# Fireflies-17/Speech-Inpainting

Measured on AMD Instinct MI355X. Metric: real-time factor (audio-sec/wall-sec) per GPU, 4 s clips @16 kHz, 200 ms mask, higher is better.
Workload: dtype encoder GEMMs and attention products: bf16 MFMA, fp32 accumulate (softmax, LayerNorm, head, arg-max in fp32); vocoder: fp16 MFMA (operands rounded to fp16, saturating), fp32 accumulate, activations stored as fp16; 1 GPU; BASELINE configs[1]: batch=32 x 4 s clips per GPU, 200 ms mask, HuBERT-base + HiFi-GAN V1; step = masked log-mel front-end -> encoder -> arg-max/splice -> vocoder on resident raw clips; global_batch=32, clip_samples=64000, mask_frames=10, parallelism=utterance-sharded x1

## Files before the change

speech_inpainting_amd/csrc/api.hip:

```cpp
#include <cmath>
#include <cstdarg>
#include <cstdio>
#include <cstdlib>
#include <cstring>
#include <map>
#include <sstream>
#include <string>
#include <vector>

#include "common.h"

namespace {

struct HostTensor {
    const float* data = nullptr;
    std::vector<long> shape;
    long numel() const { long n = 1; for (long d : shape) n *= d; return n; }
};

struct GemmW {
    size_t w = 0, w_lo = 0, bias = 0;
    int Cin = 0, N = 0, Npad = 0, ntaps = 0, groups = 1, math = 0;
    bool has_bias = false;
};

struct LayerW { GemmW qkv, out, ffn1, ffn2; size_t ln1_g, ln1_b, ln2_g, ln2_b; };
struct ConvW { GemmW g; size_t ln_g = 0, ln_b = 0; };
struct ResW { GemmW c1[SI_MAX_DIL], c2[SI_MAX_DIL]; };

struct Layout {
    size_t total = 0;
    size_t conv0_w, conv0_bias, conv0_g, conv0_b;
    std::vector<ConvW> convs;
    size_t fp_ln_g, fp_ln_b; GemmW proj;
    GemmW pos; size_t enc_ln_g, enc_ln_b;
    std::vector<LayerW> layers;
    size_t head_ln_g, head_ln_b; GemmW head;
    size_t cb_centered, cb_raw, cb_rnorm;
    GemmW pre; std::vector<GemmW> ups; std::vector<ResW> rbs;
    size_t post_w, post_b; int post_C = 0;
    int mel_ld = 0;
};

}

struct si_ctx {
    int device = 0;
    si_model_desc d{};
    char err[512] = {0};
    Layout lay;
    char* wdev = nullptr;
    bool weights_ready = false;
    bool weights_verified = false;
    std::map<std::string, long> dbg_size;
    std::map<std::string, std::pair<float*, long>> dbg_capture;
    struct ProfRec { int name; hipEvent_t a, b; double flops, bytes; };
    bool prof_on = false;
    std::string prof_filter;
    std::vector<std::string> prof_names;
    std::vector<ProfRec> prof_recs;
    std::vector<hipEvent_t> prof_pool;
    size_t prof_used = 0;
    int prof_open = -1;
    int num_cus = 0;
    std::map<const void*, size_t> dyn_lds;
    bool opt_voc_opready = true, opt_voc_res16 = true, opt_enc_opready = true, opt_att_bf16 = true, opt_enc_lingemm = true;
    bool opt_enc_posconv = true;
    int opt_ln_fuse = 1;
    int opt_voc_upsgemm = 1;
    int opt_ffn_pad = 64;
    int opt_gemmcu = 1;
    int opt_voc_chain = 1;
    int opt_voc_fuse = 1;
    char* fe_dev = nullptr;
    size_t fe_dft = 0, fe_hann = 0, fe_basis = 0, fe_lo = 0, fe_hi = 0;
    std::vector<int32_t> vl_host;
    static constexpr int VL_SLOTS = 4;
    int32_t* vl_pin[VL_SLOTS] = {nullptr, nullptr, nullptr, nullptr};
    size_t vl_pin_ints[VL_SLOTS] = {0, 0, 0, 0};
    hipEvent_t vl_ev[VL_SLOTS] = {nullptr, nullptr, nullptr, nullptr};
    int vl_next = 0;
    float* km_cnorm = nullptr;
    int km_cnorm_cap = 0;
};

static char g_create_err[512] = "";

int si_fail(si_ctx* ctx, int code, const char* fmt, ...) {
    char* dst = ctx ? ctx->err : g_create_err;
    va_list ap;
    va_start(ap, fmt);
    vsnprintf(dst, 512, fmt, ap);
    va_end(ap);
    return code;
}
int si_fail_hip(si_ctx* ctx, hipError_t e, const char* what, const char* file, int line) {
    return si_fail(ctx, SI_EHIP, "HIP error %d (%s) at %s:%d: %s", (int)e, hipGetErrorString(e), file, line, what);
}

struct TapSrc { const void* p; long n; int esize = 4; long cols = 0, ld = 0; };
static int si_tap(si_ctx* ctx, hipStream_t st, TapSrc s, const char* fmt, int a = 0, int b = 0, int c = 0) {
    if (ctx->dbg_capture.empty() && strchr(fmt, '%')) return SI_OK;
    char name[48];
    snprintf(name, sizeof(name), fmt, a, b, c);
    ctx->dbg_size[name] = s.n;
    auto it = ctx->dbg_capture.find(name);
    if (it == ctx->dbg_capture.end()) return SI_OK;
    const long m = s.n < it->second.second ? s.n : it->second.second;
    if (m <= 0) return SI_OK;
    if (s.ld > s.cols && s.cols > 0) {
        if (m / s.cols > 0)
            SI_HIP_CHECK(hipMemcpy2DAsync(it->second.first, (size_t)s.cols * s.esize, s.p, (size_t)s.ld * s.esize, (size_t)s.cols * s.esize,
                                          (size_t)(m / s.cols), hipMemcpyDeviceToDevice, st));
    } else {
        SI_HIP_CHECK(hipMemcpyAsync(it->second.first, s.p, (size_t)m * s.esize, hipMemcpyDeviceToDevice, st));
    }
    return SI_OK;
}

void si_prof_begin(si_ctx* ctx, const char* name, double flops, double bytes, hipStream_t st) {
    if (!ctx->prof_on || ctx->prof_used + 2 > ctx->prof_pool.size()) { ctx->prof_open = -1; return; }
    if (!ctx->prof_filter.empty() && ctx->prof_filter != name) { ctx->prof_open = -1; return; }
    int id = -1;
    for (size_t i = 0; i < ctx->prof_names.size(); ++i) if (ctx->prof_names[i] == name) { id = (int)i; break; }
    if (id < 0) { id = (int)ctx->prof_names.size(); ctx->prof_names.push_back(name); }
    si_ctx::ProfRec r{id, ctx->prof_pool[ctx->prof_used], ctx->prof_pool[ctx->prof_used + 1], flops, bytes};
    ctx->prof_used += 2;
    (void)hipEventRecord(r.a, st);
    ctx->prof_open = (int)ctx->prof_recs.size();
    ctx->prof_recs.push_back(r);
}
const char* si_prof_shape_name(const char* name, long M, int N, int K) {
    static const bool on = getenv("SI_PROF_SHAPES") && atoi(getenv("SI_PROF_SHAPES")) != 0;
    if (!on) return name;
    static thread_local char buf[48];
    snprintf(buf, sizeof(buf), "%s_%ldx%dx%d", name, M, N, K);
    return buf;
}
int si_ensure_dyn_lds(si_ctx* ctx, const void* kern, size_t bytes) {
    if (bytes <= 64 * 1024) return SI_OK;
    size_t& have = ctx->dyn_lds[kern];
    if (bytes > have) {
        SI_HIP_CHECK(hipFuncSetAttribute(kern, hipFuncAttributeMaxDynamicSharedMemorySize, (int)bytes));
        have = bytes;
    }
    return SI_OK;
}
int si_opt_gemmcu(const si_ctx* ctx) { return ctx->opt_gemmcu; }
int si_num_cus(si_ctx* ctx) {
    if (ctx->num_cus <= 0) {
        int n = 0;
        if (hipDeviceGetAttribute(&n, hipDeviceAttributeMultiprocessorCount, ctx->device) != hipSuccess || n <= 0) n = 256;
        ctx->num_cus = n;
    }
    return ctx->num_cus;
}
static int vl_upload(si_ctx* ctx, int32_t* dst, hipStream_t st) {
    const size_t n = ctx->vl_host.size();
    const int slot = ctx->vl_next;
    ctx->vl_next = (slot + 1) % si_ctx::VL_SLOTS;
    if (!ctx->vl_ev[slot]) SI_HIP_CHECK(hipEventCreateWithFlags(&ctx->vl_ev[slot], hipEventDisableTiming));
    else SI_HIP_CHECK(hipEventSynchronize(ctx->vl_ev[slot]));
    if (ctx->vl_pin_ints[slot] < n) {
        if (ctx->vl_pin[slot]) SI_HIP_CHECK(hipHostFree(ctx->vl_pin[slot]));
        ctx->vl_pin[slot] = nullptr; ctx->vl_pin_ints[slot] = 0;
        SI_HIP_CHECK(hipHostMalloc(reinterpret_cast<void**>(&ctx->vl_pin[slot]), std::max<size_t>(n, 4096) * sizeof(int32_t), hipHostMallocDefault));
        ctx->vl_pin_ints[slot] = std::max<size_t>(n, 4096);
    }
    memcpy(ctx->vl_pin[slot], ctx->vl_host.data(), n * sizeof(int32_t));
    SI_HIP_CHECK(hipMemcpyAsync(dst, ctx->vl_pin[slot], n * sizeof(int32_t), hipMemcpyHostToDevice, st));
    SI_HIP_CHECK(hipEventRecord(ctx->vl_ev[slot], st));
    return SI_OK;
}
void si_prof_end(si_ctx* ctx, hipStream_t st) {
    if (ctx->prof_open < 0) return;
    (void)hipEventRecord(ctx->prof_recs[ctx->prof_open].b, st);
    ctx->prof_open = -1;
}

namespace {

size_t elem_bytes(int math) { return math == SI_MATH_F32 ? 4 : 2; }

struct Planner {
    size_t cur = 0;
    size_t take(size_t bytes) { size_t o = cur; cur += (bytes + 255) / 256 * 256; return o; }
    size_t floats(size_t n) { return take(n * 4); }
    GemmW gemm(int math, int groups, int ntaps, int N, int Cin, bool bias) {
        GemmW g;
        g.math = math; g.groups = groups; g.ntaps = ntaps; g.N = N; g.Cin = Cin; g.has_bias = bias;
        g.Npad = si_round_up(N, si_pick_bn(N));
        const size_t n = (size_t)groups * ntaps * g.Npad * Cin;
        g.w = take(n * elem_bytes(math));
        if (math == SI_MATH_BF16X3) g.w_lo = take(n * 2);
        if (bias) g.bias = floats((size_t)groups * N);
        return g;
    }
};

int stage_channels(const si_ctx* ctx, int i) {
    const int real = ctx->d.up_initial_channel >> (i + 1);
    const bool r16 = ctx->opt_voc_opready && ctx->opt_voc_res16 && ctx->d.vocoder_math == SI_MATH_F16;
    return (r16 && real < 32 && real >= 4) ? 32 : real;
}

int plan_layout(si_ctx* ctx) {
    const si_model_desc& d = ctx->d;
    Layout& L = ctx->lay;
    Planner P;
    P.take(256);
    const int em = d.encoder_math, vm = d.vocoder_math;
    const int H = d.hidden_size;
    L.conv0_w = P.floats((size_t)d.conv_dim[0] * d.conv_kernel[0]);
    L.conv0_bias = d.conv_bias ? P.floats(d.conv_dim[0]) : 0;
    L.conv0_g = P.floats(d.conv_dim[0]);
    L.conv0_b = P.floats(d.conv_dim[0]);
    L.convs.clear();
    for (int i = 1; i < d.num_conv; ++i) {
        ConvW c;
        c.g = P.gemm(em, 1, d.conv_kernel[i], d.conv_dim[i], d.conv_dim[i - 1], d.conv_bias != 0);
        if (d.feat_norm_layer) { c.ln_g = P.floats(d.conv_dim[i]); c.ln_b = P.floats(d.conv_dim[i]); }
        L.convs.push_back(c);
    }
    const int CF = d.conv_dim[d.num_conv - 1];
    L.fp_ln_g = P.floats(CF); L.fp_ln_b = P.floats(CF);
    L.proj = P.gemm(em, 1, 1, H, CF, true);
    L.pos = P.gemm(em, d.pos_conv_groups, d.pos_conv_kernel, H / d.pos_conv_groups, H / d.pos_conv_groups, true);
    L.enc_ln_g = P.floats(H); L.enc_ln_b = P.floats(H);
    L.layers.clear();
    for (int l = 0; l < d.num_layers; ++l) {
        LayerW w;
        w.qkv = P.gemm(em, 1, 1, 3 * H, H, true);
        w.out = P.gemm(em, 1, 1, H, H, true);
        w.ln1_g = P.floats(H); w.ln1_b = P.floats(H);
        w.ffn1 = P.gemm(em, 1, 1, d.intermediate_size, H, true);
        w.ffn2 = P.gemm(em, 1, 1, H, d.intermediate_size, true);
        w.ln2_g = P.floats(H); w.ln2_b = P.floats(H);
        L.layers.push_back(w);
    }
    L.head_ln_g = P.floats(H); L.head_ln_b = P.floats(H);
    L.head = P.gemm(SI_MATH_F32, 1, 1, d.codebook_dim, H, true);
    L.cb_centered = P.floats((size_t)d.num_clusters * d.codebook_dim);
    L.cb_raw = P.floats((size_t)d.num_clusters * d.codebook_dim);
    L.cb_rnorm = P.floats(d.num_clusters);
    L.mel_ld = si_round_up(d.num_mels, 32);
    const int C0 = d.up_initial_channel;
    L.pre = P.gemm(vm, 1, 7, C0, L.mel_ld, true);
    L.ups.clear(); L.rbs.clear();
    int c = C0;
    for (int i = 0; i < d.num_ups; ++i) {
        const int u = d.up_rates[i], k = d.up_kernels[i], cout = stage_channels(ctx, i);
        L.ups.push_back(P.gemm(vm, 1, (k + u - 1) / u, u * cout, c, true));
        c = cout;
        for (int j = 0; j < d.num_rb; ++j) {
            ResW r;
            for (int n = 0; n < d.num_dil; ++n) {
                r.c1[n] = P.gemm(vm, 1, d.rb_kernels[j], c, c, true);
                if (d.resblock_type != 2) r.c2[n] = P.gemm(vm, 1, d.rb_kernels[j], c, c, true);
            }
            L.rbs.push_back(r);
        }
    }
    L.post_C = c;
    L.post_w = P.floats((size_t)7 * c);
    L.post_b = P.floats(1);
    L.total = P.cur;
    return SI_OK;
}

struct BlobHeader { uint32_t magic, version; uint64_t fingerprint, total; uint64_t reserved; };
constexpr uint32_t BLOB_MAGIC = 0x42574953u;
uint64_t layout_fingerprint(const si_ctx* ctx) {
    uint64_t h = 1469598103934665603ull;
    auto mix = [&](const void* p, size_t n) { const unsigned char* b = static_cast<const unsigned char*>(p); for (size_t i = 0; i < n; ++i) { h ^= b[i]; h *= 1099511628211ull; } };
    mix(&ctx->d, sizeof(ctx->d));
    const Layout& L = ctx->lay;
    const uint64_t total = L.total; mix(&total, 8);
    for (int i = 0; i < ctx->d.num_ups; ++i) { const int c = stage_channels(ctx, i); mix(&c, 4); mix(&L.ups[i].w, sizeof(size_t)); }
    mix(&L.post_w, sizeof(size_t)); mix(&L.post_C, 4); mix(&L.cb_raw, sizeof(size_t)); mix(&L.head.w, sizeof(size_t));
    return h;
}
BlobHeader blob_header(const si_ctx* ctx) { return BlobHeader{BLOB_MAGIC, (uint32_t)SI_ABI_VERSION, layout_fingerprint(ctx), (uint64_t)ctx->lay.total, 0}; }

int check_desc(si_ctx* ctx, const si_model_desc* d) {
    if (!d || d->struct_size != (int32_t)sizeof(si_model_desc))
        return si_fail(ctx, SI_EINVAL, "si_model_desc size mismatch (got %d, library expects %zu)", d ? d->struct_size : -1,
                       sizeof(si_model_desc));
    if (d->num_conv < 2 || d->num_conv > SI_MAX_CONV) return si_fail(ctx, SI_EINVAL, "num_conv=%d out of range", d->num_conv);
    if (d->num_ups < 1 || d->num_ups > SI_MAX_UPS) return si_fail(ctx, SI_EINVAL, "num_ups=%d out of range", d->num_ups);
    if (d->num_rb < 1 || d->num_rb > SI_MAX_RB || d->num_dil < 1 || d->num_dil > SI_MAX_DIL)
        return si_fail(ctx, SI_EINVAL, "resblock shape %dx%d out of range", d->num_rb, d->num_dil);
    if (d->hidden_size <= 0 || d->num_heads <= 0 || d->hidden_size != d->num_heads * 64)
        return si_fail(ctx, SI_EINVAL, "hidden_size=%d / heads=%d: the attention kernel needs head_dim 64", d->hidden_size, d->num_heads);
    if (d->pos_conv_groups <= 0 || d->hidden_size % d->pos_conv_groups || (d->hidden_size / d->pos_conv_groups) % 16)
        return si_fail(ctx, SI_EINVAL, "positional conv: hidden/groups must be a multiple of 16");
    for (int i = 0; i < d->num_conv; ++i)
        if (d->conv_dim[i] % 16 || d->conv_kernel[i] <= 0 || d->conv_stride[i] <= 0)
            return si_fail(ctx, SI_EINVAL, "conv layer %d: dim %d must be a multiple of 16", i, d->conv_dim[i]);
    if (d->hidden_size % 16 || d->intermediate_size % 16) return si_fail(ctx, SI_EINVAL, "hidden / intermediate sizes must be multiples of 16");
// ... 1526 lines not shown
```

speech_inpainting_amd/csrc/common.h:

```cpp
#pragma once
#include <hip/hip_runtime.h>
#include <stdint.h>

#include "../../include/si_hip.h"

#define SI_HIP_CHECK(expr)                                                                      \
    do {                                                                                        \
        hipError_t _e = (expr);                                                                 \
        if (_e != hipSuccess) return si_fail_hip(ctx, _e, #expr, __FILE__, __LINE__);           \
    } while (0)

int si_fail_hip(si_ctx* ctx, hipError_t e, const char* what, const char* file, int line);
int si_fail(si_ctx* ctx, int code, const char* fmt, ...);
void si_prof_begin(si_ctx* ctx, const char* name, double flops, double bytes, hipStream_t st);
void si_prof_end(si_ctx* ctx, hipStream_t st);
const char* si_prof_shape_name(const char* name, long M, int N, int K);
int si_ensure_dyn_lds(si_ctx* ctx, const void* kern, size_t bytes);
int si_num_cus(si_ctx* ctx);

typedef unsigned short bf16_t;

struct SiVlTile { int b, row0, L; };
#ifdef __HIPCC__
__device__ __forceinline__ SiVlTile si_vl_tile(const int32_t* __restrict__ lens, int B, int step, int t) {
    const int lane = (int)__builtin_amdgcn_mbcnt_hi(~0u, __builtin_amdgcn_mbcnt_lo(~0u, 0u));
    int base = 0;
    for (int s0 = 0; s0 < B; s0 += 64) {
        const int s = s0 + lane;
        const int Lb = s < B ? lens[s] : 0;
        const int nb = Lb > 0 ? (Lb + step - 1) / step : 0;
        int incl = nb;
#pragma unroll
        for (int o = 1; o < 64; o <<= 1) {
            const int v = __shfl_up(incl, o, 64);
            if (lane >= o) incl += v;
        }
        const int tot = __shfl(incl, 63, 64);
        if (t < base + tot) {
            const unsigned long long m = __ballot(base + incl > t);
            const int l = (int)__builtin_ctzll(m);
            SiVlTile r;
            r.b = s0 + l;
            r.row0 = (t - base - __shfl(incl - nb, l, 64)) * step;
            r.L = __shfl(Lb, l, 64);
            return r;
        }
        base += tot;
    }
    return SiVlTile{B, 0, 0};
}
#endif
static inline long si_vl_tiles(const int32_t* lens, int B, int step) {
    long n = 0;
    for (int b = 0; b < B; ++b) if (lens[b] > 0) n += (lens[b] + step - 1) / step;
    return n;
}

enum { SI_ACT_NONE = 0, SI_ACT_GELU = 1 };

struct TapGemmParams {
    const float* x;
    const unsigned short* x16;
    const void* w;
    const void* w_lo;
    const float* bias;
    const float* res;
    const float* res_stats; const float* res_gamma; const float* res_beta;
    const unsigned short* res16;
    int acc16;
    float* out;
    unsigned short* out16;
    float out16_slope;
    int nseg, Lin, M;
    int ldx;
    long x_seg_stride;
    int Cin;
    int N, Npad;
    int ntaps, stride, dil, pad;
    int groups;
    int ldo;
    long o_seg_stride;
    long ooff;
    long olimit;
    float pro_slope;
    int act;
    float alpha;
    int accumulate;
    double algo_macs;
    int wide_epilogue;
    int lingemm;
    const int32_t* seg_lin;
    const int32_t* seg_m;
    const int32_t* seg_orows;
    int olim_mul;
    const int32_t* seg_row_off;
    const int32_t* seg_m_host;
};

static inline int si_pick_bn(int N) { return N >= 128 ? 128 : (N > 32 ? 64 : 32); }
static inline int si_round_up(int a, int b) { return (a + b - 1) / b * b; }

int si_launch_tapgemm(si_ctx* ctx, int math, const TapGemmParams& p, hipStream_t st);

struct LinGemmParams {
    const unsigned short* x16; int x_bytes;
    int lda; long x_seg_stride;
    int nseg, M, K;
    const unsigned short* w; int w_bytes;
    int N, Cin, ntaps; long w_tap_stride;
    const float* bias; const float* res;
    const float* res_stats; const float* res_gamma; const float* res_beta;
    float* out; unsigned short* out16;
    int ldo; long o_seg_stride;
    int act;
    int xcd_rows;
    const int32_t* seg_m;
    const int32_t* seg_m_host;
    int tc_dil, tc_rows_in; float tc_slope; long tc_ooff, tc_olimit;
    const int32_t* tc_seg_lin; const int32_t* tc_seg_orows; int tc_olim_mul;
};
int si_launch_lingemm(si_ctx* ctx, const LinGemmParams& p, hipStream_t st);
int si_launch_gemmcu(si_ctx* ctx, const LinGemmParams& p, hipStream_t st);
int si_launch_gemmcu_tc(si_ctx* ctx, const TapGemmParams& p, hipStream_t st, bool always = false);
bool si_gemmcu_tc_covers(si_ctx* ctx, const TapGemmParams& p, bool always = false);
int si_opt_gemmcu(const si_ctx* ctx);

struct WaveNormParams {
    const float* wav;
    const int32_t* mask_start;
    const int32_t* mask_len;
    int B, N, L1;
    int C, K, S;
    int normalize;
    const int32_t* valid_len;
    float norm_eps;
    const double* pre_add;
    const int32_t* seg_L1;
};

struct SiSpans { const int32_t* off; const int32_t* start; const int32_t* len; };

struct SiSpanWalk {
    const int32_t* s; const int32_t* l;
    int k, n, cs, ce;
    __device__ __forceinline__ void load() {
        if (k < n) { cs = s[k]; ce = cs + l[k]; } else { cs = 0x7fffffff; ce = 0x7fffffff; }
    }
    __device__ __forceinline__ SiSpanWalk(const SiSpans& sp, int b) : s(sp.start), l(sp.len), k(sp.off[b]), n(sp.off[b + 1]) { load(); }
    __device__ __forceinline__ bool hit(int i) {
        while (i >= ce) { ++k; load(); }
        return i >= cs;
    }
    __device__ __forceinline__ bool clear(int i, int cnt) const { return i + cnt <= cs; }
};

int si_launch_wave_stats(si_ctx* ctx, const WaveNormParams& p, double* stats , hipStream_t st, const SiSpans* sp = nullptr);
int si_launch_conv0_groupnorm(si_ctx* ctx, const WaveNormParams& p, const double* stats, const float* w ,
                              const float* gamma, const float* beta, double* partials, float* affine, float* out,
                              hipStream_t st, unsigned short* out16 = nullptr ,
                              const SiSpans* sp = nullptr);
int si_launch_conv0_affine(si_ctx* ctx, const WaveNormParams& p, const double* stats, const float* w, const float* bias,
                           float* affine, float* out, hipStream_t st, const SiSpans* sp = nullptr);
size_t si_conv0_partials_bytes(int B, int N);

int si_launch_layernorm(si_ctx* ctx, const float* x, const float* add, const float* gamma, const float* beta, float* y,
                        long rows, int C, float eps, int gelu, hipStream_t st, unsigned short* y16 = nullptr, float* stats = nullptr);

int si_launch_attention(si_ctx* ctx, const float* qkv, float* out, int B, int T, int H, int heads, hipStream_t st,
                        unsigned short* out16 = nullptr, bool bf16_products = true, const int32_t* valid_frames = nullptr,
                        const int32_t* row_off = nullptr, double real_t2 = 0.0);
int si_launch_attention_bf16in(si_ctx* ctx, const unsigned short* qkv16, int B, int T, int H, int heads, hipStream_t st,
// ... 137 lines not shown
```

speech_inpainting_amd/csrc/reschain.hip:

```cpp
#include <algorithm>
#include <cstdio>
#include <cstdlib>
#include <type_traits>

#include "common.h"

typedef float f32x4 __attribute__((ext_vector_type(4)));
typedef unsigned int u32x4 __attribute__((ext_vector_type(4)));
typedef unsigned int u32x2 __attribute__((ext_vector_type(2)));
typedef _Float16 f16x8 __attribute__((ext_vector_type(8)));
typedef _Float16 f16x4 __attribute__((ext_vector_type(4)));

#ifdef RPW_TIMELINE
__device__ unsigned long long rc_tl[10];
#define RC_TL_DECL unsigned long long tl_t = wall_clock64(); unsigned long long tl_acc[8] = {0, 0, 0, 0, 0, 0, 0, 0}; unsigned long long tl_tiles = 0; unsigned long long tl_w = 0;
#define RC_TL_W0 tl_w = wall_clock64();
#define RC_TL_W1(ph) tl_acc[ph] += wall_clock64() - tl_w;
#define RC_TL(ph) { const unsigned long long n_ = wall_clock64(); tl_acc[ph] += n_ - tl_t; tl_t = n_; }
#define RC_TL_TILE ++tl_tiles;
#define RC_TL_FLUSH if (threadIdx.x == 0) { for (int q_ = 0; q_ < 8; ++q_) atomicAdd(&rc_tl[q_], tl_acc[q_]); atomicAdd(&rc_tl[8], tl_tiles); atomicAdd(&rc_tl[9], 1ull); }
extern "C" int si_debug_rc_timeline(unsigned long long* out, int reset) {
    if (hipMemcpyFromSymbol(out, HIP_SYMBOL(rc_tl), sizeof(rc_tl)) != hipSuccess) return -1;
    if (reset) { unsigned long long z[10] = {}; if (hipMemcpyToSymbol(HIP_SYMBOL(rc_tl), z, sizeof(z)) != hipSuccess) return -1; }
    return 0;
}
#else
#define RC_TL_DECL
#define RC_TL_W0
#define RC_TL_W1(ph)
#define RC_TL(ph)
#define RC_TL_TILE
#define RC_TL_FLUSH
#endif

namespace {

constexpr int RC_C = 32, RC_ROWB = 64, RC_NW = 8, RC_NT = 64 * RC_NW;
constexpr int RC_RT = 6;
constexpr int RC_R = RC_NW * RC_RT * 16;
constexpr int RC_MARG = 32;
constexpr int RC_KMAX = 11;
constexpr int RC_XBYTES = RC_R * RC_ROWB;
constexpr int RC_ABYTES = (RC_R + 2 * RC_MARG) * RC_ROWB;
constexpr int RC_WBYTES = RC_KMAX * RC_C * RC_ROWB;
constexpr int RC_LDS = RC_XBYTES + RC_ABYTES + 2 * RC_WBYTES + 6 * RC_C * 4;
constexpr int RC_WSLOTS = (RC_WBYTES / 16 + RC_NT - 1) / RC_NT;
constexpr int RC_YSLOTS = RC_R * 4 / RC_NT;
static_assert(RC_R * 4 % RC_NT == 0, "tile staging map");

__device__ __forceinline__ int rc_swz(int row) { return ((row >> 1) & 3) << 4; }

}

template <bool ACC, bool VL>
__global__ __launch_bounds__(RC_NT, 1) void reschain_kernel(const ResChainParams p) {
    extern __shared__ __attribute__((aligned(16))) char smem[];
    char* const Xs = smem;
    char* const As = smem + RC_XBYTES;
    char* const W1s = As + RC_ABYTES;
    char* const W2s = W1s + RC_WBYTES;
    float* const Bs = reinterpret_cast<float*>(W2s + RC_WBYTES);

    __builtin_amdgcn_s_setreg((0 << 11) | (23 << 6) | 1, 1);
    const int tid = threadIdx.x, lane = tid & 63, wave = tid >> 6;
    const int r16 = lane & 15, kg = lane >> 4;
    const int wm0 = wave * (RC_RT * 16);
    const int k = p.k, c = (k - 1) / 2;
    const int H = c * (p.dil[0] + p.dil[1] + p.dil[2] + 3);
    const int Rout = RC_R - 2 * H;
    const int tiles_x = (p.L + Rout - 1) / Rout;
    const int total = VL ? p.total_tiles : tiles_x * p.B;
    auto tile_of = [&](int t, int& tb, int& tm0, int& tL) {
        if constexpr (VL) { const SiVlTile v = si_vl_tile(p.lens, p.B, Rout, t); tb = v.b; tm0 = v.row0; tL = v.L; }
        else { tb = t / tiles_x; tm0 = (t - tb * tiles_x) * Rout; tL = p.L; }
    };
    const int wbytes = k * RC_C * RC_ROWB;

    u32x4 rw[RC_WSLOTS];
    auto issueW = [&](const unsigned short* w) {
        const __amdgpu_buffer_rsrc_t rs = __builtin_amdgcn_make_buffer_rsrc(const_cast<unsigned short*>(w), 0, wbytes, 0x00020000);
#pragma unroll
        for (int i = 0; i < RC_WSLOTS; ++i) rw[i] = __builtin_amdgcn_raw_buffer_load_b128(rs, (tid + i * RC_NT) * 16, 0, 0);
    };
    auto storeW = [&](char* dst) {
#pragma unroll
        for (int i = 0; i < RC_WSLOTS; ++i) {
            const int q = tid + i * RC_NT;
            if (q * 16 < wbytes) {
                const int r = q >> 2, ch = q & 3;
                *reinterpret_cast<u32x4*>(dst + r * RC_ROWB + ((ch << 4) ^ rc_swz(r))) = rw[i];
            }
        }
    };
    u32x4 ry[RC_YSLOTS];
    auto issueY = [&](int t) {
        int tb, tm0, tL;
        tile_of(t, tb, tm0, tL);
        const int g0 = tm0 - H;
        const __amdgpu_buffer_rsrc_t rs = __builtin_amdgcn_make_buffer_rsrc(const_cast<unsigned short*>(p.y16 + (long)tb * p.L * RC_C), 0, tL * RC_C * 2, 0x00020000);
#pragma unroll
        for (int i = 0; i < RC_YSLOTS; ++i) {
            const int q = tid + i * RC_NT;
            const int g = g0 + (q >> 2);
            ry[i] = __builtin_amdgcn_raw_buffer_load_b128(rs, g < 0 ? (int)0x80000000 : (g * RC_C + 8 * (q & 3)) * 2, 0, 0);
        }
    };

    if (tid < 6 * RC_C / 4) {
        const int which = tid / (RC_C / 4), c4 = (tid % (RC_C / 4)) * 4;
        const float* src = (which & 1) ? p.b2[which >> 1] : p.b1[which >> 1];
        *reinterpret_cast<f32x4*>(Bs + which * RC_C + c4) = *reinterpret_cast<const f32x4*>(src + c4);
    }
    if (tid < 2 * RC_MARG * 4) {
        const int r = tid >> 2, ch = tid & 3;
        const int row = r < RC_MARG ? r : RC_R + r;
        *reinterpret_cast<u32x4*>(As + row * RC_ROWB + (ch << 4)) = u32x4{0u, 0u, 0u, 0u};
    }
    issueW(p.w1[0]);
    issueY(blockIdx.x);
    storeW(W1s);
    issueW(p.w2[0]);

    const int preW = r16 * RC_ROWB + (rc_swz(r16) ^ (kg << 4));

    f32x4 acc[RC_RT][2];
    auto init_acc = [&](const float* bias) {
        const f32x4 b0 = *reinterpret_cast<const f32x4*>(bias + 4 * kg), b1v = *reinterpret_cast<const f32x4*>(bias + 16 + 4 * kg);
#pragma unroll
        for (int i = 0; i < RC_RT; ++i) { acc[i][0] = b0; acc[i][1] = b1v; }
    };
    const int lin0 = (wm0 + r16 + RC_MARG) * RC_ROWB + (kg << 4);
    auto el_off = [&](int i, int j, int shift) {
        const int r = wm0 + 16 * i + r16 + shift;
        const int n = 16 * j + 4 * kg;
        return r * RC_ROWB + ((((n >> 3) << 4) ^ rc_swz(r)) + 8 * (kg & 1));
    };
    auto conv = [&](const char* Wc, int dd) {
        auto load = [&](f16x8 (&y)[RC_RT], f16x8 (&w)[2], int tap) {
#ifdef RC_ABLATE_READS
            if (tap > 0) return;
#endif
            const int lin = lin0 + (tap - c) * dd * RC_ROWB;
            const char* ap = As + (lin ^ ((lin >> 3) & 0x30));
#pragma unroll
            for (int i = 0; i < RC_RT; ++i) y[i] = *reinterpret_cast<const f16x8*>(ap + i * (16 * RC_ROWB));
            const char* wp = Wc + tap * (RC_C * RC_ROWB) + preW;
#pragma unroll
            for (int j = 0; j < 2; ++j) w[j] = *reinterpret_cast<const f16x8*>(wp + j * (16 * RC_ROWB));
        };
        auto mma = [&](const f16x8 (&y)[RC_RT], const f16x8 (&w)[2]) {
#ifdef RC_ABLATE_HALF
            if (wave >= 4) return;
#endif
#ifdef RC_ABLATE_MFMA
#pragma unroll
            for (int i = 0; i < RC_RT; ++i) acc[i][0] += __builtin_bit_cast(f32x4, y[i]);
            acc[0][1] += __builtin_bit_cast(f32x4, w[0]) + __builtin_bit_cast(f32x4, w[1]);
            return;
#endif
#pragma unroll
            for (int i = 0; i < RC_RT; ++i)
#pragma unroll
                for (int j = 0; j < 2; ++j) acc[i][j] = __builtin_amdgcn_mfma_f32_16x16x32_f16(w[j], y[i], acc[i][j], 0, 0, 0);
        };
        f16x8 ya[RC_RT], wa[2], yb[RC_RT], wb[2];
        load(ya, wa, 0);
        for (int tap = 0; tap < k; tap += 2) {
            load(yb, wb, tap + 1 < k ? tap + 1 : k - 1);
            __builtin_amdgcn_sched_barrier(0);
            __builtin_amdgcn_s_setprio(1);
            mma(ya, wa);
            __builtin_amdgcn_s_setprio(0);
            __builtin_amdgcn_sched_barrier(0);
            load(ya, wa, tap + 2 < k ? tap + 2 : k - 1);
            __builtin_amdgcn_sched_barrier(0);
            if (tap + 1 < k) {
                __builtin_amdgcn_s_setprio(1);
                mma(yb, wb);
                __builtin_amdgcn_s_setprio(0);
            }
            __builtin_amdgcn_sched_barrier(0);
        }
    };

    RC_TL_DECL
    for (int tile = blockIdx.x; tile < total; tile += gridDim.x) {
        const int nxt = tile + (int)gridDim.x < total ? tile + (int)gridDim.x : tile;
        int b, tm0, Lb;
        tile_of(tile, b, tm0, Lb);
        const int g0 = tm0 - H;
        const long seg = (long)b * p.L * RC_C;
        const __amdgpu_buffer_rsrc_t orsrc = __builtin_amdgcn_make_buffer_rsrc(p.out16 + seg, 0, Lb * RC_C * 2, 0x00020000);
        const bool edge = g0 < 0 || g0 + RC_R > Lb;

#pragma unroll
        for (int i = 0; i < RC_YSLOTS; ++i) {
            const int q = tid + i * RC_NT;
            const int r = q >> 2, ch = q & 3;
            f16x8 h = __builtin_bit_cast(f16x8, ry[i]);
            *reinterpret_cast<f16x8*>(Xs + r * RC_ROWB + ((ch << 4) ^ rc_swz(r))) = h;
            h = __builtin_elementwise_max(h, h * (_Float16)0.1f);
            const int ra = r + RC_MARG;
            *reinterpret_cast<f16x8*>(As + ra * RC_ROWB + ((ch << 4) ^ rc_swz(ra))) = h;
        }
        __syncthreads();
        RC_TL(0)

        u32x2 prev[ACC ? RC_RT : 1][2];
        auto swap_halves = [&](u32x2& p0, u32x2& p1) {
#pragma unroll
            for (int q = 0; q < 2; ++q) {
                const auto r = __builtin_amdgcn_permlane16_swap(p0[q], p1[q], false, false);
                p0[q] = r[0]; p1[q] = r[1];
            }
        };
        auto chunk_off = [&](int ip, int j, int shift) {
            const int r = wm0 + 16 * (2 * ip + (kg & 1)) + r16 + shift;
            return r * RC_ROWB + ((((2 * j + (kg >> 1)) << 4)) ^ rc_swz(r));
        };
        auto epi1 = [&](auto maskc) {
            constexpr bool MASK = decltype(maskc)::value;
#pragma unroll
            for (int ip = 0; ip < RC_RT / 2; ++ip) {
                float inside[2] = {1.f, 1.f};
                if constexpr (MASK) {
#pragma unroll
                    for (int u = 0; u < 2; ++u) { const int g = g0 + wm0 + 16 * (2 * ip + u) + r16; inside[u] = (g >= 0 && g < Lb) ? 1.f : 0.f; }
                }
#pragma unroll
                for (int j = 0; j < 2; ++j) {
                    u32x2 pk[2];
#pragma unroll
                    for (int u = 0; u < 2; ++u) {
                        f16x4 hv;
#pragma unroll
                        for (int e = 0; e < 4; ++e) {
                            float v = si_lrelu01(acc[2 * ip + u][j][e]);
                            if constexpr (MASK) v *= inside[u];
                            hv[e] = (_Float16)v;
                        }
                        pk[u] = __builtin_bit_cast(u32x2, hv);
                    }
                    swap_halves(pk[0], pk[1]);
                    *reinterpret_cast<u32x4*>(As + chunk_off(ip, j, RC_MARG)) = u32x4{pk[0][0], pk[0][1], pk[1][0], pk[1][1]};
                }
            }
        };
        auto epi2 = [&](auto maskc, auto lastc) {
            constexpr bool MASK = decltype(maskc)::value, LAST = decltype(lastc)::value;
            constexpr int HP = (RC_RT / 2 + 1) / 2;
#pragma unroll
            for (int h = 0; h < 2; ++h) {
                const int ip0 = h * HP, ip1 = h == 0 ? HP : RC_RT / 2;
                f16x4 xr[HP][2][2];
#pragma unroll
                for (int ip = ip0; ip < ip1; ++ip)
#pragma unroll
                    for (int u = 0; u < 2; ++u)
#pragma unroll
                        for (int j = 0; j < 2; ++j) xr[ip - ip0][u][j] = *reinterpret_cast<const f16x4*>(Xs + el_off(2 * ip + u, j, 0));
#pragma unroll
                for (int ip = ip0; ip < ip1; ++ip) {
                    _Float16 inside[2] = {(_Float16)1.f, (_Float16)1.f};
                    if constexpr (MASK) {
#pragma unroll
                        for (int u = 0; u < 2; ++u) { const int g = g0 + wm0 + 16 * (2 * ip + u) + r16; inside[u] = (g >= 0 && g < Lb) ? (_Float16)1.f : (_Float16)0.f; }
                    }
#pragma unroll
                    for (int j = 0; j < 2; ++j) {
                        u32x2 pk[2];
#pragma unroll
                        for (int u = 0; u < 2; ++u) {
                            const int i = 2 * ip + u;
                            f16x4 xv;
#pragma unroll
                            for (int e = 0; e < 4; ++e) {
                                float v = acc[i][j][e] + (float)xr[ip - ip0][u][j][e];
                                if constexpr (LAST) {
                                    v *= p.alpha;
                                    if constexpr (ACC) v += (float)__builtin_bit_cast(f16x4, prev[i][j])[e];
                                }
                                xv[e] = (_Float16)v;
                            }
                            if constexpr (MASK) xv *= inside[u];
                            pk[u] = __builtin_bit_cast(u32x2, xv);
                        }
                        swap_halves(pk[0], pk[1]);
                        const u32x4 xc = u32x4{pk[0][0], pk[0][1], pk[1][0], pk[1][1]};
                        *reinterpret_cast<u32x4*>(Xs + chunk_off(ip, j, 0)) = xc;
                        if constexpr (!LAST) {
                            const f16x8 hx = __builtin_bit_cast(f16x8, xc);
                            *reinterpret_cast<f16x8*>(As + chunk_off(ip, j, RC_MARG)) = __builtin_elementwise_max(hx, hx * (_Float16)0.1f);
                        }
                    }
                }
            }
        };
        auto pair = [&](int pr, auto lastc) {
            constexpr bool LAST = decltype(lastc)::value;
            init_acc(Bs + (2 * pr) * RC_C);
            conv(W1s, p.dil[pr]);
            storeW(W2s);
            issueW(p.w1[LAST ? 0 : pr + 1]);
            __syncthreads();
            RC_TL(1)
            if (edge) epi1(std::true_type{}); else epi1(std::false_type{});
            __syncthreads();
            RC_TL(2)
            if constexpr (LAST) {
                issueY(nxt);
                if constexpr (ACC) {
#pragma unroll
                    for (int i = 0; i < RC_RT; ++i) {
                        const int m = wm0 + 16 * i + r16;
                        const int g = g0 + m;
                        const bool keep = m >= H && m < RC_R - H && g < Lb;
#pragma unroll
                        for (int j = 0; j < 2; ++j)
                            prev[i][j] = __builtin_amdgcn_raw_buffer_load_b64(orsrc, keep ? (g * RC_C + 16 * j + 4 * kg) * 2 : (int)0x80000000, 0, 0);
                    }
                }
            }
            init_acc(Bs + (2 * pr + 1) * RC_C);
            conv(W2s, 1);
            storeW(W1s);
            issueW(p.w2[LAST ? 0 : pr + 1]);
            __syncthreads();
            RC_TL(3)
            RC_TL_W0
            if (edge) epi2(std::true_type{}, lastc); else epi2(std::false_type{}, lastc);
            RC_TL_W1(6)
            RC_TL_W0
            __syncthreads();
            RC_TL_W1(7)
            RC_TL(4)
        };
#pragma unroll 1
        for (int pr = 0; pr < 2; ++pr) pair(pr, std::false_type{});
        pair(2, std::true_type{});

        for (int q = tid; q < Rout * 4; q += RC_NT) {
            const int r = H + (q >> 2), ch = q & 3;
            const int g = g0 + r;
            if (g < Lb) {
                const u32x4 v = *reinterpret_cast<const u32x4*>(Xs + r * RC_ROWB + ((ch << 4) ^ rc_swz(r)));
                __builtin_amdgcn_raw_buffer_store_b128(v, orsrc, (g * RC_C + 8 * ch) * 2, 0, 0);
            }
        }
        __syncthreads();
        RC_TL(5)
        RC_TL_TILE
    }
    RC_TL_FLUSH
}

int si_launch_reschain(si_ctx* ctx, int C, const ResChainParams& p, hipStream_t st) {
    if (C != RC_C || p.k < 3 || p.k > RC_KMAX || (p.k & 1) == 0 || ((long)p.L + 2048) * C * 2 >= (1L << 31) || p.B <= 0 || p.L <= 0) return 1;
    for (int i = 0; i < 3; ++i) {
        if (p.dil[i] < 1 || (p.k - 1) / 2 * p.dil[i] > RC_MARG || !p.w1[i] || !p.w2[i] || !p.b1[i] || !p.b2[i]) return 1;
    }
    const int H = (p.k - 1) / 2 * (p.dil[0] + p.dil[1] + p.dil[2] + 3);
    if (2 * H > RC_R / 4) return 1;
    if ((p.lens == nullptr) != (p.lens_host == nullptr)) return si_fail(ctx, SI_EINVAL, "reschain: ragged batches need the lengths on the device and on the host");
    const bool vl = p.lens != nullptr;
    auto kern = vl ? (p.accumulate ? reschain_kernel<true, true> : reschain_kernel<false, true>) : (p.accumulate ? reschain_kernel<true, false> : reschain_kernel<false, false>);
    if (int rc = si_ensure_dyn_lds(ctx, reinterpret_cast<const void*>(kern), RC_LDS)) return rc;
    const int Rout = RC_R - 2 * H;
    const int total = vl ? (int)si_vl_tiles(p.lens_host, p.B, Rout) : ((p.L + Rout - 1) / Rout) * p.B;
    if (total <= 0) return SI_OK;
    ResChainParams pk = p;
    pk.total_tiles = total;
    const int grid = std::min(total, si_num_cus(ctx));
    double rows = (double)p.B * p.L;
    if (vl) { rows = 0; for (int b = 0; b < p.B; ++b) rows += p.lens_host[b]; }
    const double elems = rows * C;
    si_prof_begin(ctx, p.accumulate ? "reschain_f16_c32_acc" : "reschain_f16_c32", 3 * 2.0 * 2.0 * elems * C * p.k, elems * (2.0 + 2.0 + (p.accumulate ? 2.0 : 0.0)) + 3 * 2.0 * 2.0 * p.k * C * C, st);
    hipLaunchKernelGGL(kern, dim3(grid), dim3(RC_NT), RC_LDS, st, pk);
    si_prof_end(ctx, st);
    SI_HIP_CHECK(hipGetLastError());
    return SI_OK;
}
```

Baseline: 11420 x real-time (audio-sec/wall-sec); `value` = whole-job aggregate over n_gpus, `value_per_gpu` = the per-GPU figure the metric names.

## Add two-workgroup-per-CU 4-wave reschain variant for small kernels

Templates the vocoder residual-chain kernel on wave count and row tiles, and sizes LDS from the actual kernel width instead of the maximum. A 4-wave, 7-row-tile variant that fits two workgroups per CU is chosen for k=3 when a round-count heuristic favours it and the occupancy query confirms two blocks fit. Odd row-tile counts get extra epilogue paths. The aim is better latency hiding and tail balance for the small-kernel resblocks, at the cost of more halo overhead per tile and a heuristic dispatch.

```diff
diff --git a/speech_inpainting_amd/csrc/api.hip b/speech_inpainting_amd/csrc/api.hip
--- a/speech_inpainting_amd/csrc/api.hip
+++ b/speech_inpainting_amd/csrc/api.hip
@@ -64,6 +64,7 @@
     int prof_open = -1;
     int num_cus = 0;
     std::map<const void*, size_t> dyn_lds;
+    std::map<std::pair<const void*, size_t>, int> blocks_per_cu;
     bool opt_voc_opready = true, opt_voc_res16 = true, opt_enc_opready = true, opt_att_bf16 = true, opt_enc_lingemm = true;
     bool opt_enc_posconv = true;
     int opt_ln_fuse = 1;
@@ -145,6 +146,16 @@
         have = bytes;
     }
     return SI_OK;
+}
+int si_blocks_per_cu(si_ctx* ctx, const void* kern, int threads, size_t lds) {
+    const auto key = std::make_pair(kern, lds);
+    auto it = ctx->blocks_per_cu.find(key);
+    if (it == ctx->blocks_per_cu.end()) {
+        int n = 0;
+        SI_HIP_CHECK(hipOccupancyMaxActiveBlocksPerMultiprocessor(&n, kern, threads, lds));
+        it = ctx->blocks_per_cu.emplace(key, n).first;
+    }
+    return it->second;
 }
 int si_opt_gemmcu(const si_ctx* ctx) { return ctx->opt_gemmcu; }
 int si_num_cus(si_ctx* ctx) {
diff --git a/speech_inpainting_amd/csrc/common.h b/speech_inpainting_amd/csrc/common.h
--- a/speech_inpainting_amd/csrc/common.h
+++ b/speech_inpainting_amd/csrc/common.h
@@ -17,6 +17,7 @@
 const char* si_prof_shape_name(const char* name, long M, int N, int K);
 int si_ensure_dyn_lds(si_ctx* ctx, const void* kern, size_t bytes);
 int si_num_cus(si_ctx* ctx);
+int si_blocks_per_cu(si_ctx* ctx, const void* kern, int threads, size_t lds);
 
 typedef unsigned short bf16_t;
 
diff --git a/speech_inpainting_amd/csrc/reschain.hip b/speech_inpainting_amd/csrc/reschain.hip
--- a/speech_inpainting_amd/csrc/reschain.hip
+++ b/speech_inpainting_amd/csrc/reschain.hip
@@ -12,16 +12,19 @@
 typedef _Float16 f16x4 __attribute__((ext_vector_type(4)));
 
 #ifdef RPW_TIMELINE
-__device__ unsigned long long rc_tl[10];
+#define RC_TL_ROWS 6
+#define RC_TL_COLS 12
+__device__ unsigned long long rc_tl[RC_TL_ROWS][RC_TL_COLS];
 #define RC_TL_DECL unsigned long long tl_t = wall_clock64(); unsigned long long tl_acc[8] = {0, 0, 0, 0, 0, 0, 0, 0}; unsigned long long tl_tiles = 0; unsigned long long tl_w = 0;
 #define RC_TL_W0 tl_w = wall_clock64();
 #define RC_TL_W1(ph) tl_acc[ph] += wall_clock64() - tl_w;
 #define RC_TL(ph) { const unsigned long long n_ = wall_clock64(); tl_acc[ph] += n_ - tl_t; tl_t = n_; }
 #define RC_TL_TILE ++tl_tiles;
-#define RC_TL_FLUSH if (threadIdx.x == 0) { for (int q_ = 0; q_ < 8; ++q_) atomicAdd(&rc_tl[q_], tl_acc[q_]); atomicAdd(&rc_tl[8], tl_tiles); atomicAdd(&rc_tl[9], 1ull); }
+#define RC_TL_FLUSH if (threadIdx.x == 0) { unsigned long long* row_ = rc_tl[(p.k - 1) / 2 < RC_TL_ROWS ? (p.k - 1) / 2 : RC_TL_ROWS - 1]; \
+    for (int q_ = 0; q_ < 8; ++q_) atomicAdd(&row_[q_], tl_acc[q_]); atomicAdd(&row_[8], tl_tiles); atomicAdd(&row_[9], 1ull); row_[10] = NW; row_[11] = RT; }
 extern "C" int si_debug_rc_timeline(unsigned long long* out, int reset) {
     if (hipMemcpyFromSymbol(out, HIP_SYMBOL(rc_tl), sizeof(rc_tl)) != hipSuccess) return -1;
-    if (reset) { unsigned long long z[10] = {}; if (hipMemcpyToSymbol(HIP_SYMBOL(rc_tl), z, sizeof(z)) != hipSuccess) return -1; }
+    if (reset) { unsigned long long z[RC_TL_ROWS][RC_TL_COLS] = {}; if (hipMemcpyToSymbol(HIP_SYMBOL(rc_tl), z, sizeof(z)) != hipSuccess) return -1; }
     return 0;
 }
 #else
@@ -35,37 +38,53 @@
 
 namespace {
 
-constexpr int RC_C = 32, RC_ROWB = 64, RC_NW = 8, RC_NT = 64 * RC_NW;
-constexpr int RC_RT = 6;
-constexpr int RC_R = RC_NW * RC_RT * 16;
+constexpr int RC_C = 32, RC_ROWB = 64;
 constexpr int RC_MARG = 32;
 constexpr int RC_KMAX = 11;
-constexpr int RC_XBYTES = RC_R * RC_ROWB;
-constexpr int RC_ABYTES = (RC_R + 2 * RC_MARG) * RC_ROWB;
-constexpr int RC_WBYTES = RC_KMAX * RC_C * RC_ROWB;
-constexpr int RC_LDS = RC_XBYTES + RC_ABYTES + 2 * RC_WBYTES + 6 * RC_C * 4;
-constexpr int RC_WSLOTS = (RC_WBYTES / 16 + RC_NT - 1) / RC_NT;
-constexpr int RC_YSLOTS = RC_R * 4 / RC_NT;
-static_assert(RC_R * 4 % RC_NT == 0, "tile staging map");
+constexpr int RC_CU_LDS = 160 * 1024;
+
+template <int NW, int RT>
+struct RcGeom {
+    static constexpr int NT = 64 * NW;
+    static constexpr int R = NW * RT * 16;
+    static constexpr int XBYTES = R * RC_ROWB;
+    static constexpr int ABYTES = (R + 2 * RC_MARG) * RC_ROWB;
+    static constexpr int WG_PER_CU = NW == 4 ? 2 : 1;
+    static constexpr int wbytes(int k) { return k * RC_C * RC_ROWB; }
+    static constexpr int lds(int k) { return XBYTES + ABYTES + 2 * wbytes(k) + 6 * RC_C * 4; }
+    static constexpr int kmax() { int k = RC_KMAX; while (k > 1 && lds(k) > RC_CU_LDS / WG_PER_CU) k -= 2; return k; }
+    static constexpr int KMAX = kmax();
+    static constexpr int WSLOTS = (wbytes(KMAX) / 16 + NT - 1) / NT;
+    static constexpr int YSLOTS = R * 4 / NT;
+    static_assert(R * 4 % NT == 0 && 2 * RC_MARG * 4 <= NT && 6 * RC_C / 4 <= NT, "staging maps");
+    static_assert(XBYTES % 1024 == 0, "the operand image keeps the swizzle's alignment");
+    static_assert(KMAX >= 3 && lds(KMAX) * WG_PER_CU <= RC_CU_LDS, "LDS");
+};
+static_assert(RcGeom<8, 6>::KMAX == 11 && RcGeom<8, 6>::lds(11) == 148224 && RcGeom<8, 6>::WSLOTS == 3, "the 8-wave form is laid out as before");
+static_assert(RcGeom<4, 7>::KMAX == 3 && RcGeom<4, 7>::lds(3) == 74496 && RcGeom<4, 5>::KMAX == 7 && RcGeom<4, 5>::lds(7) == 74496, "two workgroups per CU");
 
 __device__ __forceinline__ int rc_swz(int row) { return ((row >> 1) & 3) << 4; }
 
 }
 
-template <bool ACC, bool VL>
-__global__ __launch_bounds__(RC_NT, 1) void reschain_kernel(const ResChainParams p) {
+template <int NW, int RT, bool ACC, bool VL>
+__global__ __launch_bounds__(64 * NW, NW == 4 ? 2 : 1) void reschain_kernel(const ResChainParams p) {
+    using G = RcGeom<NW, RT>;
+    constexpr int RC_NT = G::NT, RC_RT = RT, RC_R = G::R, RC_XBYTES = G::XBYTES, RC_ABYTES = G::ABYTES;
+    constexpr int RC_WSLOTS = G::WSLOTS, RC_YSLOTS = G::YSLOTS;
+    const int k = p.k, c = (k - 1) / 2;
+    const int wbytes = G::wbytes(k);
     extern __shared__ __attribute__((aligned(16))) char smem[];
     char* const Xs = smem;
     char* const As = smem + RC_XBYTES;
     char* const W1s = As + RC_ABYTES;
-    char* const W2s = W1s + RC_WBYTES;
-    float* const Bs = reinterpret_cast<float*>(W2s + RC_WBYTES);
+    char* const W2s = W1s + wbytes;
+    float* const Bs = reinterpret_cast<float*>(W2s + wbytes);
 
     __builtin_amdgcn_s_setreg((0 << 11) | (23 << 6) | 1, 1);
     const int tid = threadIdx.x, lane = tid & 63, wave = tid >> 6;
     const int r16 = lane & 15, kg = lane >> 4;
     const int wm0 = wave * (RC_RT * 16);
-    const int k = p.k, c = (k - 1) / 2;
     const int H = c * (p.dil[0] + p.dil[1] + p.dil[2] + 3);
     const int Rout = RC_R - 2 * H;
     const int tiles_x = (p.L + Rout - 1) / Rout;
@@ -74,7 +93,6 @@
         if constexpr (VL) { const SiVlTile v = si_vl_tile(p.lens, p.B, Rout, t); tb = v.b; tm0 = v.row0; tL = v.L; }
         else { tb = t / tiles_x; tm0 = (t - tb * tiles_x) * Rout; tL = p.L; }
     };
-    const int wbytes = k * RC_C * RC_ROWB;
 
     u32x4 rw[RC_WSLOTS];
     auto issueW = [&](const unsigned short* w) {
@@ -218,6 +236,10 @@
             const int r = wm0 + 16 * (2 * ip + (kg & 1)) + r16 + shift;
             return r * RC_ROWB + ((((2 * j + (kg >> 1)) << 4)) ^ rc_swz(r));
         };
+        auto odd_off = [&](int shift) {
+            const int r = wm0 + 16 * (RC_RT - 1) + r16 + shift;
+            return r * RC_ROWB + (((2 * (kg & 1) + (kg >> 1)) << 4) ^ rc_swz(r));
+        };
         auto epi1 = [&](auto maskc) {
             constexpr bool MASK = decltype(maskc)::value;
 #pragma unroll
@@ -245,10 +267,51 @@
                     *reinterpret_cast<u32x4*>(As + chunk_off(ip, j, RC_MARG)) = u32x4{pk[0][0], pk[0][1], pk[1][0], pk[1][1]};
                 }
             }
+            if constexpr (RC_RT & 1) {
+                constexpr int i = RC_RT - 1;
+                float inside = 1.f;
+                if constexpr (MASK) { const int g = g0 + wm0 + 16 * i + r16; inside = (g >= 0 && g < Lb) ? 1.f : 0.f; }
+                u32x2 pk[2];
+#pragma unroll
+                for (int j = 0; j < 2; ++j) {
+                    f16x4 hv;
+#pragma unroll
+                    for (int e = 0; e < 4; ++e) {
+                        float v = si_lrelu01(acc[i][j][e]);
+                        if constexpr (MASK) v *= inside;
+                        hv[e] = (_Float16)v;
+                    }
+                    pk[j] = __builtin_bit_cast(u32x2, hv);
+                }
+                swap_halves(pk[0], pk[1]);
+                *reinterpret_cast<u32x4*>(As + odd_off(RC_MARG)) = u32x4{pk[0][0], pk[0][1], pk[1][0], pk[1][1]};
+            }
         };
         auto epi2 = [&](auto maskc, auto lastc) {
             constexpr bool MASK = decltype(maskc)::value, LAST = decltype(lastc)::value;
             constexpr int HP = (RC_RT / 2 + 1) / 2;
+            auto xnew = [&](int i, int j, const f16x4& x, _Float16 inside) {
+                f16x4 xv;
+#pragma unroll
+                for (int e = 0; e < 4; ++e) {
+                    float v = acc[i][j][e] + (float)x[e];
+                    if constexpr (LAST) {
+                        v *= p.alpha;
+                        if constexpr (ACC) v += (float)__builtin_bit_cast(f16x4, prev[i][j])[e];
+                    }
+                    xv[e] = (_Float16)v;
+                }
+                if constexpr (MASK) xv *= inside;
+                return __builtin_bit_cast(u32x2, xv);
+            };
+            auto put = [&](int off0, int offA, const u32x2 (&pk)[2]) {
+                const u32x4 xc = u32x4{pk[0][0], pk[0][1], pk[1][0], pk[1][1]};
+                *reinterpret_cast<u32x4*>(Xs + off0) = xc;
+                if constexpr (!LAST) {
+                    const f16x8 hx = __builtin_bit_cast(f16x8, xc);
+                    *reinterpret_cast<f16x8*>(As + offA) = __builtin_elementwise_max(hx, hx * (_Float16)0.1f);
+                }
+            };
 #pragma unroll
             for (int h = 0; h < 2; ++h) {
                 const int ip0 = h * HP, ip1 = h == 0 ? HP : RC_RT / 2;
@@ -259,6 +322,13 @@
                     for (int u = 0; u < 2; ++u)
 #pragma unroll
                         for (int j = 0; j < 2; ++j) xr[ip - ip0][u][j] = *reinterpret_cast<const f16x4*>(Xs + el_off(2 * ip + u, j, 0));
+                f16x4 xo[2];
+                if constexpr (RC_RT & 1) {
+                    if (h == 1) {
+#pragma unroll
+                        for (int j = 0; j < 2; ++j) xo[j] = *reinterpret_cast<const f16x4*>(Xs + el_off(RC_RT - 1, j, 0));
+                    }
+                }
 #pragma unroll
                 for (int ip = ip0; ip < ip1; ++ip) {
                     _Float16 inside[2] = {(_Float16)1.f, (_Float16)1.f};
@@ -270,28 +340,21 @@
                     for (int j = 0; j < 2; ++j) {
                         u32x2 pk[2];
 #pragma unroll
-                        for (int u = 0; u < 2; ++u) {
-                            const int i = 2 * ip + u;
-                            f16x4 xv;
-#pragma unroll
-                            for (int e = 0; e < 4; ++e) {
-                                float v = acc[i][j][e] + (float)xr[ip - ip0][u][j][e];
-                                if constexpr (LAST) {
-                                    v *= p.alpha;
-                                    if constexpr (ACC) v += (float)__builtin_bit_cast(f16x4, prev[i][j])[e];
-                                }
-                                xv[e] = (_Float16)v;
-                            }
-                            if constexpr (MASK) xv *= inside[u];
-                            pk[u] = __builtin_bit_cast(u32x2, xv);
-                        }
+                        for (int u = 0; u < 2; ++u) pk[u] = xnew(2 * ip + u, j, xr[ip - ip0][u][j], inside[u]);
                         swap_halves(pk[0], pk[1]);
-                        const u32x4 xc = u32x4{pk[0][0], pk[0][1], pk[1][0], pk[1][1]};
-                        *reinterpret_cast<u32x4*>(Xs + chunk_off(ip, j, 0)) = xc;
-                        if constexpr (!LAST) {
-                            const f16x8 hx = __builtin_bit_cast(f16x8, xc);
-                            *reinterpret_cast<f16x8*>(As + chunk_off(ip, j, RC_MARG)) = __builtin_elementwise_max(hx, hx * (_Float16)0.1f);
-                        }
+                        put(chunk_off(ip, j, 0), chunk_off(ip, j, RC_MARG), pk);
+                    }
+                }
+                if constexpr (RC_RT & 1) {
+                    if (h == 1) {
+                        constexpr int i = RC_RT - 1;
+                        _Float16 inside = (_Float16)1.f;
+                        if constexpr (MASK) { const int g = g0 + wm0 + 16 * i + r16; inside = (g >= 0 && g < Lb) ? (_Float16)1.f : (_Float16)0.f; }
+                        u32x2 pk[2];
+#pragma unroll
+                        for (int j = 0; j < 2; ++j) pk[j] = xnew(i, j, xo[j], inside);
+                        swap_halves(pk[0], pk[1]);
+                        put(odd_off(0), odd_off(RC_MARG), pk);
                     }
                 }
             }
@@ -354,29 +417,77 @@
     RC_TL_FLUSH
 }
 
+namespace {
+
+template <int NW, int RT>
+const void* rc_kernel(bool acc, bool vl) {
+    return vl ? (acc ? reinterpret_cast<const void*>(reschain_kernel<NW, RT, true, true>) : reinterpret_cast<const void*>(reschain_kernel<NW, RT, false, true>))
+              : (acc ? reinterpret_cast<const void*>(reschain_kernel<NW, RT, true, false>) : reinterpret_cast<const void*>(reschain_kernel<NW, RT, false, false>));
+}
+
+long rc_tiles(const ResChainParams& p, int Rout) {
+    return p.lens ? si_vl_tiles(p.lens_host, p.B, Rout) : (long)((p.L + Rout - 1) / Rout) * p.B;
+}
+
+struct RcPlan { bool ok; long tiles, rounds; };
+template <int NW, int RT>
+RcPlan rc_plan(const ResChainParams& p, int H, int cus) {
+    using G = RcGeom<NW, RT>;
+    if (p.k > G::KMAX || 2 * H > G::R / 4) return RcPlan{false, 0, 0};
+    const long tiles = rc_tiles(p, G::R - 2 * H), slots = (long)cus * G::WG_PER_CU;
+    return RcPlan{true, tiles, (tiles + slots - 1) / slots};
+}
+
+template <int NW, int RT>
+int rc_launch(si_ctx* ctx, const ResChainParams& p, int H, hipStream_t st) {
+    using G = RcGeom<NW, RT>;
+    const void* kern = rc_kernel<NW, RT>(p.accumulate != 0, p.lens != nullptr);
+    const int lds = G::lds(p.k);
+    if (int rc = si_ensure_dyn_lds(ctx, kern, lds)) return rc;
+    const long total = rc_tiles(p, G::R - 2 * H);
+    if (total <= 0) return SI_OK;
+    ResChainParams pk = p;
+    pk.total_tiles = (int)total;
+    const int grid = (int)std::min<long>(total, (long)si_num_cus(ctx) * G::WG_PER_CU);
+    double rows = (double)p.B * p.L;
+    if (p.lens) { rows = 0; for (int b = 0; b < p.B; ++b) rows += p.lens_host[b]; }
+    const double elems = rows * RC_C;
+    si_prof_begin(ctx, p.accumulate ? "reschain_f16_c32_acc" : "reschain_f16_c32", 3 * 2.0 * 2.0 * elems * RC_C * p.k, elems * (2.0 + 2.0 + (p.accumulate ? 2.0 : 0.0)) + 3 * 2.0 * 2.0 * p.k * RC_C * RC_C, st);
+    void* args[] = {&pk};
+    const hipError_t e = hipLaunchKernel(kern, dim3(grid), dim3(G::NT), args, lds, st);
+    si_prof_end(ctx, st);
+    SI_HIP_CHECK(e);
+    SI_HIP_CHECK(hipGetLastError());
+    return SI_OK;
+}
+
+template <int NW, int RT>
+int rc_try_two(si_ctx* ctx, const ResChainParams& p, int H, const RcPlan& one, hipStream_t st) {
+    using G = RcGeom<NW, RT>;
+    const RcPlan two = rc_plan<NW, RT>(p, H, si_num_cus(ctx));
+    if (!two.ok || two.rounds * RT * 13 >= one.rounds * 6 * 20) return 0;
+    const void* kern = rc_kernel<NW, RT>(p.accumulate != 0, p.lens != nullptr);
+    if (int rc = si_ensure_dyn_lds(ctx, kern, G::lds(p.k))) return rc;
+    const int per_cu = si_blocks_per_cu(ctx, kern, G::NT, G::lds(p.k));
+    if (per_cu < 0) return per_cu;
+    if (per_cu != G::WG_PER_CU) return 0;
+    const int rc = rc_launch<NW, RT>(ctx, p, H, st);
+    return rc < 0 ? rc : 1;
+}
+
+}
+
 int si_launch_reschain(si_ctx* ctx, int C, const ResChainParams& p, hipStream_t st) {
     if (C != RC_C || p.k < 3 || p.k > RC_KMAX || (p.k & 1) == 0 || ((long)p.L + 2048) * C * 2 >= (1L << 31) || p.B <= 0 || p.L <= 0) return 1;
     for (int i = 0; i < 3; ++i) {
         if (p.dil[i] < 1 || (p.k - 1) / 2 * p.dil[i] > RC_MARG || !p.w1[i] || !p.w2[i] || !p.b1[i] || !p.b2[i]) return 1;
     }
     const int H = (p.k - 1) / 2 * (p.dil[0] + p.dil[1] + p.dil[2] + 3);
-    if (2 * H > RC_R / 4) return 1;
+    const RcPlan one = rc_plan<8, 6>(p, H, si_num_cus(ctx));
+    if (!one.ok) return 1;
     if ((p.lens == nullptr) != (p.lens_host == nullptr)) return si_fail(ctx, SI_EINVAL, "reschain: ragged batches need the lengths on the device and on the host");
-    const bool vl = p.lens != nullptr;
-    auto kern = vl ? (p.accumulate ? reschain_kernel<true, true> : reschain_kernel<false, true>) : (p.accumulate ? reschain_kernel<true, false> : reschain_kernel<false, false>);
-    if (int rc = si_ensure_dyn_lds(ctx, reinterpret_cast<const void*>(kern), RC_LDS)) return rc;
-    const int Rout = RC_R - 2 * H;
-    const int total = vl ? (int)si_vl_tiles(p.lens_host, p.B, Rout) : ((p.L + Rout - 1) / Rout) * p.B;
-    if (total <= 0) return SI_OK;
-    ResChainParams pk = p;
-    pk.total_tiles = total;
-    const int grid = std::min(total, si_num_cus(ctx));
-    double rows = (double)p.B * p.L;
-    if (vl) { rows = 0; for (int b = 0; b < p.B; ++b) rows += p.lens_host[b]; }
-    const double elems = rows * C;
-    si_prof_begin(ctx, p.accumulate ? "reschain_f16_c32_acc" : "reschain_f16_c32", 3 * 2.0 * 2.0 * elems * C * p.k, elems * (2.0 + 2.0 + (p.accumulate ? 2.0 : 0.0)) + 3 * 2.0 * 2.0 * p.k * C * C, st);
-    hipLaunchKernelGGL(kern, dim3(grid), dim3(RC_NT), RC_LDS, st, pk);
-    si_prof_end(ctx, st);
-    SI_HIP_CHECK(hipGetLastError());
-    return SI_OK;
-}
+#ifndef RC_ONE_WORKGROUP
+    if (p.k <= RcGeom<4, 7>::KMAX) { if (int rc = rc_try_two<4, 7>(ctx, p, H, one, st)) return rc < 0 ? rc : SI_OK; }
+#endif
+    return rc_launch<8, 6>(ctx, p, H, st);
+}
```

New measurement: 11110 x real-time (audio-sec/wall-sec); `value` = whole-job aggregate over n_gpus, `value_per_gpu` = the per-GPU figure the metric names. 0.973x the previous value.
